# stanfordnlp/mac-network

Measured on NVIDIA H100. Metric: mac_reasoning_steps_per_sec, higher is better.
Workload: dtype bf16

## Files before the change

mac_network_b200/csrc/read_step.cuh:

```cuda
#pragma once
#include "tc_gemm.cuh"

namespace mac {

constexpr int RS_D = 512;
constexpr int RS_BM = 64;
constexpr int RS_KB = RS_D / TC_BK;
constexpr int RS_BLK = RS_BM * TC_BK * 2;
constexpr int RS_A_BYTES = RS_KB * RS_BLK;
constexpr int RS_B_HALF = 256 * TC_BK * 2;
constexpr int RS_W_BYTES = 2 * RS_B_HALF;
constexpr int RS_STAGE = RS_W_BYTES + RS_BLK;
constexpr int RS_STAGES = 2;
constexpr int RS_Q_SLOT = RS_KB;
constexpr int RS_SLOTS = RS_Q_SLOT + 1 + RS_KB;
constexpr int RS_CONSUMERS = 256;
constexpr int RS_THREADS = RS_CONSUMERS + 32;
constexpr int RS_SMEM_BYTES = RS_A_BYTES + RS_STAGES * RS_STAGE + 1024  + 64  +
                              2 * RS_BM * 4  + 2 * RS_D * 4  +
                              2 * RS_D * 4 ;
static_assert(RS_SMEM_BYTES <= 232448, "over the sm_90 per-block shared memory opt-in limit");
static_assert(RS_STAGE % 1024 == 0 && RS_W_BYTES % 1024 == 0, "swizzled operands need 1024-byte alignment");

__device__ __forceinline__ float bf16lo(uint32_t w) { return __uint_as_float(w << 16); }
__device__ __forceinline__ float bf16hi(uint32_t w) { return __uint_as_float(w & 0xffff0000u); }

__device__ __forceinline__ void wgmma_bf16_n256(float (&d)[128], uint64_t adesc, uint64_t bdesc, uint32_t accum) {
  asm volatile(
      "{\n\t.reg .pred p;\n\t"
      "setp.ne.b32 p, %130, 0;\n\t"
      "wgmma.mma_async.sync.aligned.m64n256k16.f32.bf16.bf16 "
      "{%0, %1, %2, %3, %4, %5, %6, %7, %8, %9, %10, %11, %12, %13, %14, %15, %16, %17, %18, %19, %20, %21, %22, %23, %24, %25, %26, %27, %28, %29, %30, %31, %32, %33, %34, %35, %36, %37, %38, %39, %40, %41, %42, %43, %44, %45, %46, %47, %48, %49, %50, %51, %52, %53, %54, %55, %56, %57, %58, %59, %60, %61, %62, %63, %64, %65, %66, %67, %68, %69, %70, %71, %72, %73, %74, %75, %76, %77, %78, %79, %80, %81, %82, %83, %84, %85, %86, %87, %88, %89, %90, %91, %92, %93, %94, %95, %96, %97, %98, %99, %100, %101, %102, %103, %104, %105, %106, %107, %108, %109, %110, %111, %112, %113, %114, %115, %116, %117, %118, %119, %120, %121, %122, %123, %124, %125, %126, %127}, %128, %129, p, 1, 1, 0, 0;\n\t}"
      : "+f"(d[0]), "+f"(d[1]), "+f"(d[2]), "+f"(d[3]), "+f"(d[4]), "+f"(d[5]), "+f"(d[6]), "+f"(d[7]), "+f"(d[8]), "+f"(d[9]), "+f"(d[10]), "+f"(d[11]), "+f"(d[12]), "+f"(d[13]), "+f"(d[14]), "+f"(d[15]), "+f"(d[16]), "+f"(d[17]), "+f"(d[18]), "+f"(d[19]), "+f"(d[20]), "+f"(d[21]), "+f"(d[22]), "+f"(d[23]), "+f"(d[24]), "+f"(d[25]), "+f"(d[26]), "+f"(d[27]), "+f"(d[28]), "+f"(d[29]), "+f"(d[30]), "+f"(d[31]), "+f"(d[32]), "+f"(d[33]), "+f"(d[34]), "+f"(d[35]), "+f"(d[36]), "+f"(d[37]), "+f"(d[38]), "+f"(d[39]), "+f"(d[40]), "+f"(d[41]), "+f"(d[42]), "+f"(d[43]), "+f"(d[44]), "+f"(d[45]), "+f"(d[46]), "+f"(d[47]), "+f"(d[48]), "+f"(d[49]), "+f"(d[50]), "+f"(d[51]), "+f"(d[52]), "+f"(d[53]), "+f"(d[54]), "+f"(d[55]), "+f"(d[56]), "+f"(d[57]), "+f"(d[58]), "+f"(d[59]), "+f"(d[60]), "+f"(d[61]), "+f"(d[62]), "+f"(d[63]), "+f"(d[64]), "+f"(d[65]), "+f"(d[66]), "+f"(d[67]), "+f"(d[68]), "+f"(d[69]), "+f"(d[70]), "+f"(d[71]), "+f"(d[72]), "+f"(d[73]), "+f"(d[74]), "+f"(d[75]), "+f"(d[76]), "+f"(d[77]), "+f"(d[78]), "+f"(d[79]), "+f"(d[80]), "+f"(d[81]), "+f"(d[82]), "+f"(d[83]), "+f"(d[84]), "+f"(d[85]), "+f"(d[86]), "+f"(d[87]), "+f"(d[88]), "+f"(d[89]), "+f"(d[90]), "+f"(d[91]), "+f"(d[92]), "+f"(d[93]), "+f"(d[94]), "+f"(d[95]), "+f"(d[96]), "+f"(d[97]), "+f"(d[98]), "+f"(d[99]), "+f"(d[100]), "+f"(d[101]), "+f"(d[102]), "+f"(d[103]), "+f"(d[104]), "+f"(d[105]), "+f"(d[106]), "+f"(d[107]), "+f"(d[108]), "+f"(d[109]), "+f"(d[110]), "+f"(d[111]), "+f"(d[112]), "+f"(d[113]), "+f"(d[114]), "+f"(d[115]), "+f"(d[116]), "+f"(d[117]), "+f"(d[118]), "+f"(d[119]), "+f"(d[120]), "+f"(d[121]), "+f"(d[122]), "+f"(d[123]), "+f"(d[124]), "+f"(d[125]), "+f"(d[126]), "+f"(d[127])
      : "l"(adesc), "l"(bdesc), "r"(accum));
}
inline bool read_step_supported(int B, int N, int d) {
  return d == RS_D && N >= 1 && N <= 256 && B >= 1 && B < (1 << 22);
}

struct ReadStepParams {
  int M, N;
  const float* y;
  const float* ctrl;
  const float* bm2;
  const float* wr;
  float* logits;
};

__device__ __forceinline__ void rs_consumer_bar() { asm volatile("bar.sync 1, %0;" ::"n"(RS_CONSUMERS) : "memory"); }

__global__ void __launch_bounds__(RS_THREADS, 1)
read_step_kernel(const __grid_constant__ CUtensorMap map_p, const __grid_constant__ CUtensorMap map_q,
                 const __grid_constant__ CUtensorMap map_w1, const __grid_constant__ CUtensorMap map_w2,
                 const ReadStepParams p) {
  extern __shared__ unsigned char smem_dyn[];
  const uint32_t base_u32 = smem_u32(smem_dyn);
  unsigned char* a_tile = smem_dyn + ((1024u - (base_u32 & 1023u)) & 1023u);
  unsigned char* b_ring = a_tile + RS_A_BYTES;
  uint64_t* full = reinterpret_cast<uint64_t*>(b_ring + RS_STAGES * RS_STAGE);
  uint64_t* empty = full + RS_STAGES;
  float* s_lg = reinterpret_cast<float*>(full + 8);
  float* s_ctrl = s_lg + 2 * RS_BM;
  float* s_bm2 = s_ctrl + 2 * RS_D;
  float* s_wr = s_bm2 + RS_D;

  const int warp = threadIdx.x >> 5, lane = threadIdx.x & 31;
  const int row0 = blockIdx.x * RS_BM;
  const int s_lo = row0 / p.N;

  if (threadIdx.x == RS_CONSUMERS) {
    tma_prefetch_desc(&map_p);
    tma_prefetch_desc(&map_q);
    tma_prefetch_desc(&map_w1);
    tma_prefetch_desc(&map_w2);
    for (int i = 0; i < RS_STAGES; ++i) {
      mbar_init(&full[i], 1);
      mbar_init(&empty[i], RS_CONSUMERS / 32);
    }
    fence_mbar_init();
  }
  __syncthreads();

  if (warp == RS_CONSUMERS / 32) {
    if (elect_one()) {
      for (int j = 0; j < RS_SLOTS; ++j) {
        const int s = j % RS_STAGES;
        mbar_wait(&empty[s], ((j / RS_STAGES) & 1) ^ 1);
        unsigned char* dst = b_ring + s * RS_STAGE;
        if (j == RS_Q_SLOT) {
          mbar_expect_tx(&full[s], RS_A_BYTES);
          for (int kb = 0; kb < RS_KB; ++kb) tma_load_2d(dst + kb * RS_BLK, &map_q, kb * TC_BK, row0, &full[s]);
          continue;
        }
        const bool g1 = j < RS_Q_SLOT;
        mbar_expect_tx(&full[s], g1 ? RS_W_BYTES + RS_BLK : RS_W_BYTES);
        const CUtensorMap* m = g1 ? &map_w1 : &map_w2;
        const int k0 = (g1 ? j : j - RS_Q_SLOT - 1) * TC_BK;
        if (g1) tma_load_2d(dst + RS_W_BYTES, &map_p, k0, row0, &full[s]);
        tma_load_2d(dst, m, k0, 0, &full[s]);
        tma_load_2d(dst + RS_B_HALF, m, k0, 256, &full[s]);
      }
    }
    return;
  }

  const int tid = threadIdx.x;
  const int g = warp >> 2;
  const int rl = 16 * (warp & 3) + (lane >> 2);
  const int cq = 256 * g + 2 * (lane & 3);
  const int prow = tid >> 3;
  const int poff = prow * 128 + (tid & 7) * 16;
  const int pcol = ((tid & 7) ^ (prow & 7)) << 3;
  for (int i = tid; i < RS_D; i += RS_CONSUMERS) {
    s_bm2[i] = __ldg(p.bm2 + i);
    s_wr[i] = __ldg(p.wr + i);
  }
  float acc[128];
  const int last_row = min(p.M, row0 + RS_BM) - 1;
  const int nsamp = last_row / p.N - s_lo + 1;
  for (int q = 0; q < min(nsamp, 2); ++q)
    for (int i = tid; i < RS_D; i += RS_CONSUMERS) s_ctrl[q * RS_D + i] = __ldg(p.ctrl + (size_t)(s_lo + q) * RS_D + i);
  int yoff[2];
#pragma unroll
  for (int u = 0; u < 2; ++u) yoff[u] = min(row0 + prow + 32 * u, p.M - 1) / p.N * RS_D + pcol;

  for (int j = 0; j < RS_KB; ++j) {
    const int s = j % RS_STAGES;
    unsigned char* stage = b_ring + s * RS_STAGE;
    float4 y0[2], y1[2];
#pragma unroll
    for (int u = 0; u < 2; ++u) {
      y0[u] = *reinterpret_cast<const float4*>(p.y + yoff[u] + j * TC_BK);
      y1[u] = *reinterpret_cast<const float4*>(p.y + yoff[u] + j * TC_BK + 4);
    }
    mbar_wait(&full[s], (j / RS_STAGES) & 1);
#pragma unroll
    for (int u = 0; u < 2; ++u) {
      uint4* c = reinterpret_cast<uint4*>(stage + RS_W_BYTES + poff + u * 32 * 128);
      const uint4 v = *c;
      *c = make_uint4(pack_bf16(bf16lo(v.x) * y0[u].x, bf16hi(v.x) * y0[u].y), pack_bf16(bf16lo(v.y) * y0[u].z, bf16hi(v.y) * y0[u].w),
                      pack_bf16(bf16lo(v.z) * y1[u].x, bf16hi(v.z) * y1[u].y), pack_bf16(bf16lo(v.w) * y1[u].z, bf16hi(v.w) * y1[u].w));
    }
    fence_proxy_async();
    rs_consumer_bar();
    const uint64_t adesc = make_sw128_kmajor_desc(smem_u32(stage + RS_W_BYTES));
    const uint64_t bdesc = make_sw128_kmajor_desc(smem_u32(stage + g * RS_B_HALF));
    wgmma_fence();
#pragma unroll
    for (int k = 0; k < TC_BK / 16; ++k) wgmma_bf16_n256(acc, adesc + 2 * k, bdesc + 2 * k, (j || k) ? 1u : 0u);
    wgmma_commit();
    wgmma_wait<1>();
    wgmma_hold(acc);
    if (j && lane == 0) mbar_arrive(&empty[(j - 1) % RS_STAGES]);
  }
  wgmma_wait<0>();
  wgmma_hold(acc);
  if (lane == 0) mbar_arrive(&empty[(RS_KB - 1) % RS_STAGES]);

  constexpr int qs = RS_Q_SLOT % RS_STAGES;
  const unsigned char* q_tile = b_ring + qs * RS_STAGE;
  mbar_wait(&full[qs], (RS_Q_SLOT / RS_STAGES) & 1);
#pragma unroll
  for (int h = 0; h < 2; ++h) {
    const int r = rl + 8 * h, row = row0 + r;
#pragma unroll
    for (int j = 0; j < 32; ++j) {
      const int n = cq + 8 * j;
      const int kb = n >> 6, c = (n & 63) >> 3;
      const int off = kb * RS_BLK + r * 128 + ((c ^ (r & 7)) << 4) + (n & 7) * 2;
      const uint32_t q = *reinterpret_cast<const uint32_t*>(q_tile + off);
      const uint32_t hv = row < p.M ? pack_bf16(elu_fast(acc[4 * j + 2 * h] + bf16lo(q)), elu_fast(acc[4 * j + 2 * h + 1] + bf16hi(q)))
                                    : 0u;
      *reinterpret_cast<uint32_t*>(a_tile + off) = hv;
    }
  }
  fence_proxy_async();
  rs_consumer_bar();
  if (lane == 0) mbar_arrive(&empty[qs]);

  const uint32_t a_u = smem_u32(a_tile);
  for (int j = 0; j < RS_KB; ++j) {
    const int jj = RS_Q_SLOT + 1 + j, s = jj % RS_STAGES;
    mbar_wait(&full[s], (jj / RS_STAGES) & 1);
    const uint64_t adesc = make_sw128_kmajor_desc(a_u + j * RS_BLK);
    const uint64_t bdesc = make_sw128_kmajor_desc(smem_u32(b_ring + s * RS_STAGE + g * RS_B_HALF));
    wgmma_fence();
#pragma unroll
    for (int k = 0; k < TC_BK / 16; ++k) wgmma_bf16_n256(acc, adesc + 2 * k, bdesc + 2 * k, (j || k) ? 1u : 0u);
    wgmma_commit();
    wgmma_wait<1>();
    wgmma_hold(acc);
    if (j && lane == 0) mbar_arrive(&empty[(jj - 1) % RS_STAGES]);
  }
  wgmma_wait<0>();
  wgmma_hold(acc);
  if (lane == 0) mbar_arrive(&empty[(RS_SLOTS - 1) % RS_STAGES]);

#pragma unroll
  for (int h = 0; h < 2; ++h) {
    const int r = rl + 8 * h, row = row0 + r;
    const int s = min(row, p.M - 1) / p.N;
    const float* crow = s - s_lo < 2 ? s_ctrl + (s - s_lo) * RS_D : p.ctrl + (size_t)s * RS_D;
    float part = 0.f;
#pragma unroll
    for (int j = 0; j < 32; ++j) {
      const int n = cq + 8 * j;
      const float2 cc = *reinterpret_cast<const float2*>(crow + n);
      const float2 bb = *reinterpret_cast<const float2*>(s_bm2 + n);
      const float2 ww = *reinterpret_cast<const float2*>(s_wr + n);
      const float t0 = elu_fast((acc[4 * j + 2 * h] + bb.x) * cc.x);
      const float t1 = elu_fast((acc[4 * j + 2 * h + 1] + bb.y) * cc.y);
      part = fmaf(t0, ww.x, part);
      part = fmaf(t1, ww.y, part);
    }
    part += __shfl_xor_sync(0xffffffffu, part, 1);
    part += __shfl_xor_sync(0xffffffffu, part, 2);
    if ((lane & 3) == 0) s_lg[g * RS_BM + r] = part;
  }
  rs_consumer_bar();
  if (tid < RS_BM && row0 + tid < p.M) p.logits[row0 + tid] = s_lg[tid] + s_lg[RS_BM + tid];
}

inline int read_step_launch(const void* inv, const void* kb_bf16, const float* y, const float* control,
                            const mac_read_weights* w, float* att, float* info, int B, int N, int d, cudaStream_t stream) {
  if (!read_step_supported(B, N, d)) return MAC_ERR_UNSUPPORTED;
  if (!inv || !kb_bf16 || !y || !control || !w->Wm_bf16 || !w->Wm2_bf16 || !att || !info) return MAC_ERR_INVALID;
  const int M = B * N;
  const TcReadScratch s = tc_read_scratch(const_cast<void*>(inv), B, N, d);
  CUtensorMap mp, mq, mw1, mw2;
  int st = make_tmap_2d(&mp, s.P, 1, (uint64_t)M, (uint64_t)d, (uint64_t)d * 2, RS_BM, TC_BK, 1);
  if (st != MAC_OK) return st;
  st = make_tmap_2d(&mq, s.Q, 1, (uint64_t)M, (uint64_t)d, (uint64_t)d * 2, RS_BM, TC_BK, 1);
  if (st != MAC_OK) return st;
  st = make_tmap_2d(&mw1, w->Wm_bf16, 1, (uint64_t)d, (uint64_t)d, (uint64_t)2 * d * 2, 256, TC_BK, 1);
  if (st != MAC_OK) return st;
  st = make_tmap_2d(&mw2, w->Wm2_bf16, 1, (uint64_t)d, (uint64_t)d, (uint64_t)d * 2, 256, TC_BK, 1);
  if (st != MAC_OK) return st;
  ReadStepParams p{};
  p.M = M; p.N = N; p.y = y; p.ctrl = control; p.bm2 = w->bm2; p.wr = w->wr; p.logits = s.parts;
  MAC_CUDA_TRY(cudaFuncSetAttribute(read_step_kernel, cudaFuncAttributeMaxDynamicSharedMemorySize, RS_SMEM_BYTES));
  read_step_kernel<<<(M + RS_BM - 1) / RS_BM, RS_THREADS, RS_SMEM_BYTES, stream>>>(mp, mq, mw1, mw2, p);
  MAC_LAUNCH_CHECK();
  return mac_kb_attend_fwd(s.parts, 1, w->br, kb_bf16, 1, att, info, B, N, d, stream);
}

}
```

Baseline: 17630.

## Retile fused read-step kernel to 128-row blocks with per-warpgroup rows and register rebalancing

The fused read-step GEMM kernel now handles 128 rows per block, with each consumer warpgroup owning 64 rows across all 512 output columns. Before, each warpgroup owned 256 columns of a 64-row tile, so each weight tile loaded from memory now serves twice as many rows. The P operand is loaded once into a persistent A tile with per-block barriers, and the weight ring is restaged as a 3-deep ring of 256-column halves. It adds setmaxnreg producer/consumer register reallocation, keeps the first-half hidden activations in registers, and prefetches y one step ahead. The cost is a larger block with heavy register pressure (232 registers per consumer thread), fewer blocks for small M, and control/bias/weight vectors read from global memory instead of shared memory.

```diff
diff --git a/mac_network_b200/csrc/read_step.cuh b/mac_network_b200/csrc/read_step.cuh
--- a/mac_network_b200/csrc/read_step.cuh
+++ b/mac_network_b200/csrc/read_step.cuh
@@ -9,18 +9,31 @@
 constexpr int RS_BLK = RS_BM * TC_BK * 2;
 constexpr int RS_A_BYTES = RS_KB * RS_BLK;
 constexpr int RS_B_HALF = 256 * TC_BK * 2;
-constexpr int RS_W_BYTES = 2 * RS_B_HALF;
-constexpr int RS_STAGE = RS_W_BYTES + RS_BLK;
-constexpr int RS_STAGES = 2;
-constexpr int RS_Q_SLOT = RS_KB;
-constexpr int RS_SLOTS = RS_Q_SLOT + 1 + RS_KB;
 constexpr int RS_CONSUMERS = 256;
 constexpr int RS_THREADS = RS_CONSUMERS + 32;
-constexpr int RS_SMEM_BYTES = RS_A_BYTES + RS_STAGES * RS_STAGE + 1024  + 64  +
-                              2 * RS_BM * 4  + 2 * RS_D * 4  +
-                              2 * RS_D * 4 ;
-static_assert(RS_SMEM_BYTES <= 232448, "over the sm_90 per-block shared memory opt-in limit");
-static_assert(RS_STAGE % 1024 == 0 && RS_W_BYTES % 1024 == 0, "swizzled operands need 1024-byte alignment");
+
+constexpr int RS128_BM = 128;
+constexpr int RS128_BLK = RS128_BM * TC_BK * 2;
+constexpr int RS128_A_BYTES = RS_KB * RS128_BLK;
+constexpr int RS128_STAGE = RS_B_HALF;
+constexpr int RS128_STAGES = 3;
+constexpr int RS128_Q0 = RS_KB;
+constexpr int RS128_G1B = RS128_Q0 + 2;
+constexpr int RS128_Q1 = RS128_G1B + RS_KB;
+constexpr int RS128_G2A = RS128_Q1 + 2;
+constexpr int RS128_G2B = RS128_G2A + RS_KB;
+constexpr int RS128_SLOTS = RS128_G2B + RS_KB;
+constexpr int RS128_CONSUMERS = 256;
+constexpr int RS128_THREADS = RS128_CONSUMERS + 128;
+constexpr int RS128_SMEM_BYTES = RS128_A_BYTES + RS128_STAGES * RS128_STAGE + 1024  +
+                                 8 * (RS_KB + 2 * RS128_STAGES) ;
+static_assert(RS128_SMEM_BYTES <= 232448, "over the sm_90 per-block shared memory opt-in limit");
+static_assert(RS128_BLK % 1024 == 0 && RS128_STAGE % 1024 == 0 && (RS128_BM / 2) * 128 % 1024 == 0,
+              "swizzled operands need 1024-byte alignment");
+static_assert(2 * RS128_BLK == RS128_STAGE, "a ring slot holds two Q blocks");
+constexpr int RS128_PRODUCER_REGS = 40;
+constexpr int RS128_CONSUMER_REGS = 232;
+static_assert(RS128_PRODUCER_REGS + 2 * RS128_CONSUMER_REGS <= 3 * (65536 / RS128_THREADS / 8 * 8), "register budget");
 
 __device__ __forceinline__ float bf16lo(uint32_t w) { return __uint_as_float(w << 16); }
 __device__ __forceinline__ float bf16hi(uint32_t w) { return __uint_as_float(w & 0xffff0000u); }
@@ -49,176 +62,232 @@
 
 __device__ __forceinline__ void rs_consumer_bar() { asm volatile("bar.sync 1, %0;" ::"n"(RS_CONSUMERS) : "memory"); }
 
-__global__ void __launch_bounds__(RS_THREADS, 1)
+__device__ __forceinline__ void rs128_wg_bar(int g) { asm volatile("bar.sync %0, 128;" ::"r"(1 + g) : "memory"); }
+
+__device__ __forceinline__ void rs128_gemm_half(float (&acc)[128], uint32_t a_u, uint32_t ring_u, uint64_t* full,
+                                                uint64_t* empty, int t0, int lane) {
+  for (int j = 0; j < RS_KB; ++j) {
+    const int t = t0 + j, s = t % RS128_STAGES;
+    mbar_wait(&full[s], (t / RS128_STAGES) & 1);
+    const uint64_t adesc = make_sw128_kmajor_desc(a_u + j * RS128_BLK);
+    const uint64_t bdesc = make_sw128_kmajor_desc(ring_u + s * RS128_STAGE);
+    wgmma_fence();
+#pragma unroll
+    for (int k = 0; k < TC_BK / 16; ++k) wgmma_bf16_n256(acc, adesc + 2 * k, bdesc + 2 * k, (j || k) ? 1u : 0u);
+    wgmma_commit();
+    wgmma_wait<1>();
+    wgmma_hold(acc);
+    if (j && lane == 0) mbar_arrive(&empty[(t - 1) % RS128_STAGES]);
+  }
+  wgmma_wait<0>();
+  wgmma_hold(acc);
+  if (lane == 0) mbar_arrive(&empty[(t0 + RS_KB - 1) % RS128_STAGES]);
+}
+
+__device__ __forceinline__ int rs128_sw_off(int r, int n, int blk) {
+  return (n >> 6) * blk + r * 128 + ((((n & 63) >> 3) ^ (r & 7)) << 4) + (n & 7) * 2;
+}
+
+__global__ void __launch_bounds__(RS128_THREADS, 1)
 read_step_kernel(const __grid_constant__ CUtensorMap map_p, const __grid_constant__ CUtensorMap map_q,
                  const __grid_constant__ CUtensorMap map_w1, const __grid_constant__ CUtensorMap map_w2,
                  const ReadStepParams p) {
   extern __shared__ unsigned char smem_dyn[];
   const uint32_t base_u32 = smem_u32(smem_dyn);
   unsigned char* a_tile = smem_dyn + ((1024u - (base_u32 & 1023u)) & 1023u);
-  unsigned char* b_ring = a_tile + RS_A_BYTES;
-  uint64_t* full = reinterpret_cast<uint64_t*>(b_ring + RS_STAGES * RS_STAGE);
-  uint64_t* empty = full + RS_STAGES;
-  float* s_lg = reinterpret_cast<float*>(full + 8);
-  float* s_ctrl = s_lg + 2 * RS_BM;
-  float* s_bm2 = s_ctrl + 2 * RS_D;
-  float* s_wr = s_bm2 + RS_D;
+  unsigned char* ring = a_tile + RS128_A_BYTES;
+  uint64_t* pfull = reinterpret_cast<uint64_t*>(ring + RS128_STAGES * RS128_STAGE);
+  uint64_t* full = pfull + RS_KB;
+  uint64_t* empty = full + RS128_STAGES;
 
   const int warp = threadIdx.x >> 5, lane = threadIdx.x & 31;
-  const int row0 = blockIdx.x * RS_BM;
-  const int s_lo = row0 / p.N;
-
-  if (threadIdx.x == RS_CONSUMERS) {
+  const int row0 = blockIdx.x * RS128_BM;
+
+  if (threadIdx.x == RS128_CONSUMERS) {
     tma_prefetch_desc(&map_p);
     tma_prefetch_desc(&map_q);
     tma_prefetch_desc(&map_w1);
     tma_prefetch_desc(&map_w2);
-    for (int i = 0; i < RS_STAGES; ++i) {
+    for (int i = 0; i < RS_KB; ++i) mbar_init(&pfull[i], 1);
+    for (int i = 0; i < RS128_STAGES; ++i) {
       mbar_init(&full[i], 1);
-      mbar_init(&empty[i], RS_CONSUMERS / 32);
+      mbar_init(&empty[i], RS128_CONSUMERS / 32);
     }
     fence_mbar_init();
   }
   __syncthreads();
 
-  if (warp == RS_CONSUMERS / 32) {
-    if (elect_one()) {
-      for (int j = 0; j < RS_SLOTS; ++j) {
-        const int s = j % RS_STAGES;
-        mbar_wait(&empty[s], ((j / RS_STAGES) & 1) ^ 1);
-        unsigned char* dst = b_ring + s * RS_STAGE;
-        if (j == RS_Q_SLOT) {
-          mbar_expect_tx(&full[s], RS_A_BYTES);
-          for (int kb = 0; kb < RS_KB; ++kb) tma_load_2d(dst + kb * RS_BLK, &map_q, kb * TC_BK, row0, &full[s]);
-          continue;
+  if (warp >= RS128_CONSUMERS / 32) {
+    asm volatile("setmaxnreg.dec.sync.aligned.u32 %0;" ::"n"(RS128_PRODUCER_REGS));
+    if (warp == RS128_CONSUMERS / 32 && elect_one()) {
+      auto load_p = [&](int j) {
+        mbar_expect_tx(&pfull[j], RS128_BLK);
+        tma_load_2d(a_tile + j * RS128_BLK, &map_p, j * TC_BK, row0, &pfull[j]);
+      };
+      for (int t = 0; t < RS128_SLOTS; ++t) {
+        if (t < RS128_STAGES) load_p(t);
+        else if (t == RS128_STAGES)
+          for (int j = RS128_STAGES; j < RS_KB; ++j) load_p(j);
+        const int s = t % RS128_STAGES;
+        mbar_wait(&empty[s], ((t / RS128_STAGES) & 1) ^ 1);
+        unsigned char* dst = ring + s * RS128_STAGE;
+        mbar_expect_tx(&full[s], RS128_STAGE);
+        if (t < RS128_G2A) {
+          const int half = t >= RS128_G1B, u = t - half * RS128_G1B;
+          if (u < RS_KB) {
+            tma_load_2d(dst, &map_w1, u * TC_BK, 256 * half, &full[s]);
+          } else {
+            const int kb = 4 * half + 2 * (u - RS_KB);
+            tma_load_2d(dst, &map_q, kb * TC_BK, row0, &full[s]);
+            tma_load_2d(dst + RS128_BLK, &map_q, (kb + 1) * TC_BK, row0, &full[s]);
+          }
+        } else {
+          const int half = t >= RS128_G2B, u = t - (half ? RS128_G2B : RS128_G2A);
+          tma_load_2d(dst, &map_w2, u * TC_BK, 256 * half, &full[s]);
         }
-        const bool g1 = j < RS_Q_SLOT;
-        mbar_expect_tx(&full[s], g1 ? RS_W_BYTES + RS_BLK : RS_W_BYTES);
-        const CUtensorMap* m = g1 ? &map_w1 : &map_w2;
-        const int k0 = (g1 ? j : j - RS_Q_SLOT - 1) * TC_BK;
-        if (g1) tma_load_2d(dst + RS_W_BYTES, &map_p, k0, row0, &full[s]);
-        tma_load_2d(dst, m, k0, 0, &full[s]);
-        tma_load_2d(dst + RS_B_HALF, m, k0, 256, &full[s]);
       }
     }
     return;
   }
 
-  const int tid = threadIdx.x;
+  asm volatile("setmaxnreg.inc.sync.aligned.u32 %0;" ::"n"(RS128_CONSUMER_REGS));
   const int g = warp >> 2;
+  const int wt = threadIdx.x & 127;
   const int rl = 16 * (warp & 3) + (lane >> 2);
-  const int cq = 256 * g + 2 * (lane & 3);
-  const int prow = tid >> 3;
-  const int poff = prow * 128 + (tid & 7) * 16;
-  const int pcol = ((tid & 7) ^ (prow & 7)) << 3;
-  for (int i = tid; i < RS_D; i += RS_CONSUMERS) {
-    s_bm2[i] = __ldg(p.bm2 + i);
-    s_wr[i] = __ldg(p.wr + i);
-  }
+  const int cq = 2 * (lane & 3);
+  const int rowg = row0 + 64 * g;
+  unsigned char* a_wg = a_tile + g * (RS128_BM / 2) * 128;
+  const uint32_t a_u = smem_u32(a_wg), ring_u = smem_u32(ring);
+  const int prow = wt >> 3;
+  const int poff = prow * 128 + (wt & 7) * 16;
+  const int pcol = ((wt & 7) ^ (prow & 7)) << 3;
+  int yoff[4];
+#pragma unroll
+  for (int u = 0; u < 4; ++u) yoff[u] = min(rowg + prow + 16 * u, p.M - 1) / p.N * RS_D + pcol;
+
   float acc[128];
-  const int last_row = min(p.M, row0 + RS_BM) - 1;
-  const int nsamp = last_row / p.N - s_lo + 1;
-  for (int q = 0; q < min(nsamp, 2); ++q)
-    for (int i = tid; i < RS_D; i += RS_CONSUMERS) s_ctrl[q * RS_D + i] = __ldg(p.ctrl + (size_t)(s_lo + q) * RS_D + i);
-  int yoff[2];
-#pragma unroll
-  for (int u = 0; u < 2; ++u) yoff[u] = min(row0 + prow + 32 * u, p.M - 1) / p.N * RS_D + pcol;
-
-  for (int j = 0; j < RS_KB; ++j) {
-    const int s = j % RS_STAGES;
-    unsigned char* stage = b_ring + s * RS_STAGE;
-    float4 y0[2], y1[2];
-#pragma unroll
-    for (int u = 0; u < 2; ++u) {
+  float4 y0[4], y1[4];
+  auto load_y = [&](int j) {
+#pragma unroll
+    for (int u = 0; u < 4; ++u) {
       y0[u] = *reinterpret_cast<const float4*>(p.y + yoff[u] + j * TC_BK);
       y1[u] = *reinterpret_cast<const float4*>(p.y + yoff[u] + j * TC_BK + 4);
     }
-    mbar_wait(&full[s], (j / RS_STAGES) & 1);
-#pragma unroll
-    for (int u = 0; u < 2; ++u) {
-      uint4* c = reinterpret_cast<uint4*>(stage + RS_W_BYTES + poff + u * 32 * 128);
+  };
+  load_y(0);
+  for (int j = 0; j < RS_KB; ++j) {
+    const int s = j % RS128_STAGES;
+    mbar_wait(&pfull[j], 0);
+#pragma unroll
+    for (int u = 0; u < 4; ++u) {
+      uint4* c = reinterpret_cast<uint4*>(a_wg + j * RS128_BLK + poff + u * 16 * 128);
       const uint4 v = *c;
       *c = make_uint4(pack_bf16(bf16lo(v.x) * y0[u].x, bf16hi(v.x) * y0[u].y), pack_bf16(bf16lo(v.y) * y0[u].z, bf16hi(v.y) * y0[u].w),
                       pack_bf16(bf16lo(v.z) * y1[u].x, bf16hi(v.z) * y1[u].y), pack_bf16(bf16lo(v.w) * y1[u].z, bf16hi(v.w) * y1[u].w));
     }
     fence_proxy_async();
-    rs_consumer_bar();
-    const uint64_t adesc = make_sw128_kmajor_desc(smem_u32(stage + RS_W_BYTES));
-    const uint64_t bdesc = make_sw128_kmajor_desc(smem_u32(stage + g * RS_B_HALF));
+    rs128_wg_bar(g);
+    mbar_wait(&full[s], (j / RS128_STAGES) & 1);
+    const uint64_t adesc = make_sw128_kmajor_desc(a_u + j * RS128_BLK);
+    const uint64_t bdesc = make_sw128_kmajor_desc(ring_u + s * RS128_STAGE);
     wgmma_fence();
 #pragma unroll
     for (int k = 0; k < TC_BK / 16; ++k) wgmma_bf16_n256(acc, adesc + 2 * k, bdesc + 2 * k, (j || k) ? 1u : 0u);
     wgmma_commit();
+    if (j + 1 < RS_KB) load_y(j + 1);
     wgmma_wait<1>();
     wgmma_hold(acc);
-    if (j && lane == 0) mbar_arrive(&empty[(j - 1) % RS_STAGES]);
+    if (j && lane == 0) mbar_arrive(&empty[(j - 1) % RS128_STAGES]);
   }
   wgmma_wait<0>();
   wgmma_hold(acc);
-  if (lane == 0) mbar_arrive(&empty[(RS_KB - 1) % RS_STAGES]);
-
-  constexpr int qs = RS_Q_SLOT % RS_STAGES;
-  const unsigned char* q_tile = b_ring + qs * RS_STAGE;
-  mbar_wait(&full[qs], (RS_Q_SLOT / RS_STAGES) & 1);
+  if (lane == 0) mbar_arrive(&empty[(RS_KB - 1) % RS128_STAGES]);
+
+  uint32_t h0[64];
+#pragma unroll
+  for (int q = 0; q < 2; ++q) {
+    const int t = RS128_Q0 + q, s = t % RS128_STAGES;
+    mbar_wait(&full[s], (t / RS128_STAGES) & 1);
+    const unsigned char* q_tile = ring + s * RS128_STAGE + g * (RS128_BM / 2) * 128 - 2 * q * RS128_BLK;
+#pragma unroll
+    for (int h = 0; h < 2; ++h) {
+      const int r = rl + 8 * h;
+      const bool live = rowg + r < p.M;
+#pragma unroll
+      for (int j = 16 * q; j < 16 * q + 16; ++j) {
+        const uint32_t qv = *reinterpret_cast<const uint32_t*>(q_tile + rs128_sw_off(r, cq + 8 * j, RS128_BLK));
+        h0[2 * j + h] = live ? pack_bf16(elu_fast(acc[4 * j + 2 * h] + bf16lo(qv)), elu_fast(acc[4 * j + 2 * h + 1] + bf16hi(qv)))
+                             : 0u;
+      }
+    }
+    __syncwarp();
+    if (lane == 0) mbar_arrive(&empty[s]);
+  }
+
+  rs128_gemm_half(acc, a_u, ring_u, full, empty, RS128_G1B, lane);
+
+  rs128_wg_bar(g);
 #pragma unroll
   for (int h = 0; h < 2; ++h) {
-    const int r = rl + 8 * h, row = row0 + r;
-#pragma unroll
-    for (int j = 0; j < 32; ++j) {
-      const int n = cq + 8 * j;
-      const int kb = n >> 6, c = (n & 63) >> 3;
-      const int off = kb * RS_BLK + r * 128 + ((c ^ (r & 7)) << 4) + (n & 7) * 2;
-      const uint32_t q = *reinterpret_cast<const uint32_t*>(q_tile + off);
-      const uint32_t hv = row < p.M ? pack_bf16(elu_fast(acc[4 * j + 2 * h] + bf16lo(q)), elu_fast(acc[4 * j + 2 * h + 1] + bf16hi(q)))
-                                    : 0u;
-      *reinterpret_cast<uint32_t*>(a_tile + off) = hv;
-    }
+    const int r = rl + 8 * h;
+#pragma unroll
+    for (int j = 0; j < 32; ++j) *reinterpret_cast<uint32_t*>(a_wg + rs128_sw_off(r, cq + 8 * j, RS128_BLK)) = h0[2 * j + h];
+  }
+#pragma unroll
+  for (int q = 0; q < 2; ++q) {
+    const int t = RS128_Q1 + q, s = t % RS128_STAGES;
+    mbar_wait(&full[s], (t / RS128_STAGES) & 1);
+    const unsigned char* q_tile = ring + s * RS128_STAGE + g * (RS128_BM / 2) * 128 - 2 * q * RS128_BLK;
+#pragma unroll
+    for (int h = 0; h < 2; ++h) {
+      const int r = rl + 8 * h;
+      const bool live = rowg + r < p.M;
+#pragma unroll
+      for (int j = 16 * q; j < 16 * q + 16; ++j) {
+        const int n = cq + 8 * j;
+        const uint32_t qv = *reinterpret_cast<const uint32_t*>(q_tile + rs128_sw_off(r, n, RS128_BLK));
+        *reinterpret_cast<uint32_t*>(a_wg + rs128_sw_off(r, 256 + n, RS128_BLK)) =
+            live ? pack_bf16(elu_fast(acc[4 * j + 2 * h] + bf16lo(qv)), elu_fast(acc[4 * j + 2 * h + 1] + bf16hi(qv))) : 0u;
+      }
+    }
+    __syncwarp();
+    if (lane == 0) mbar_arrive(&empty[s]);
   }
   fence_proxy_async();
-  rs_consumer_bar();
-  if (lane == 0) mbar_arrive(&empty[qs]);
-
-  const uint32_t a_u = smem_u32(a_tile);
-  for (int j = 0; j < RS_KB; ++j) {
-    const int jj = RS_Q_SLOT + 1 + j, s = jj % RS_STAGES;
-    mbar_wait(&full[s], (jj / RS_STAGES) & 1);
-    const uint64_t adesc = make_sw128_kmajor_desc(a_u + j * RS_BLK);
-    const uint64_t bdesc = make_sw128_kmajor_desc(smem_u32(b_ring + s * RS_STAGE + g * RS_B_HALF));
-    wgmma_fence();
-#pragma unroll
-    for (int k = 0; k < TC_BK / 16; ++k) wgmma_bf16_n256(acc, adesc + 2 * k, bdesc + 2 * k, (j || k) ? 1u : 0u);
-    wgmma_commit();
-    wgmma_wait<1>();
-    wgmma_hold(acc);
-    if (j && lane == 0) mbar_arrive(&empty[(jj - 1) % RS_STAGES]);
-  }
-  wgmma_wait<0>();
-  wgmma_hold(acc);
-  if (lane == 0) mbar_arrive(&empty[(RS_SLOTS - 1) % RS_STAGES]);
-
+  rs128_wg_bar(g);
+
+  float part[2][2];
+#pragma unroll
+  for (int half = 0; half < 2; ++half) {
+    rs128_gemm_half(acc, a_u, ring_u, full, empty, half ? RS128_G2B : RS128_G2A, lane);
+#pragma unroll
+    for (int h = 0; h < 2; ++h) {
+      const int row = rowg + rl + 8 * h;
+      const float* crow = p.ctrl + (size_t)(min(row, p.M - 1) / p.N) * RS_D + 256 * half;
+      const float* bm2 = p.bm2 + 256 * half;
+      const float* wr = p.wr + 256 * half;
+      float s = 0.f;
+#pragma unroll
+      for (int j = 0; j < 32; ++j) {
+        const int n = cq + 8 * j;
+        const float2 cc = __ldg(reinterpret_cast<const float2*>(crow + n));
+        const float2 bb = __ldg(reinterpret_cast<const float2*>(bm2 + n));
+        const float2 ww = __ldg(reinterpret_cast<const float2*>(wr + n));
+        const float t0 = elu_fast((acc[4 * j + 2 * h] + bb.x) * cc.x);
+        const float t1 = elu_fast((acc[4 * j + 2 * h + 1] + bb.y) * cc.y);
+        s = fmaf(t0, ww.x, s);
+        s = fmaf(t1, ww.y, s);
+      }
+      s += __shfl_xor_sync(0xffffffffu, s, 1);
+      s += __shfl_xor_sync(0xffffffffu, s, 2);
+      part[half][h] = s;
+    }
+  }
 #pragma unroll
   for (int h = 0; h < 2; ++h) {
-    const int r = rl + 8 * h, row = row0 + r;
-    const int s = min(row, p.M - 1) / p.N;
-    const float* crow = s - s_lo < 2 ? s_ctrl + (s - s_lo) * RS_D : p.ctrl + (size_t)s * RS_D;
-    float part = 0.f;
-#pragma unroll
-    for (int j = 0; j < 32; ++j) {
-      const int n = cq + 8 * j;
-      const float2 cc = *reinterpret_cast<const float2*>(crow + n);
-      const float2 bb = *reinterpret_cast<const float2*>(s_bm2 + n);
-      const float2 ww = *reinterpret_cast<const float2*>(s_wr + n);
-      const float t0 = elu_fast((acc[4 * j + 2 * h] + bb.x) * cc.x);
-      const float t1 = elu_fast((acc[4 * j + 2 * h + 1] + bb.y) * cc.y);
-      part = fmaf(t0, ww.x, part);
-      part = fmaf(t1, ww.y, part);
-    }
-    part += __shfl_xor_sync(0xffffffffu, part, 1);
-    part += __shfl_xor_sync(0xffffffffu, part, 2);
-    if ((lane & 3) == 0) s_lg[g * RS_BM + r] = part;
-  }
-  rs_consumer_bar();
-  if (tid < RS_BM && row0 + tid < p.M) p.logits[row0 + tid] = s_lg[tid] + s_lg[RS_BM + tid];
+    const int row = rowg + rl + 8 * h;
+    if ((lane & 3) == 0 && row < p.M) p.logits[row] = part[0][h] + part[1][h];
+  }
 }
 
 inline int read_step_launch(const void* inv, const void* kb_bf16, const float* y, const float* control,
@@ -228,9 +297,9 @@
   const int M = B * N;
   const TcReadScratch s = tc_read_scratch(const_cast<void*>(inv), B, N, d);
   CUtensorMap mp, mq, mw1, mw2;
-  int st = make_tmap_2d(&mp, s.P, 1, (uint64_t)M, (uint64_t)d, (uint64_t)d * 2, RS_BM, TC_BK, 1);
+  int st = make_tmap_2d(&mp, s.P, 1, (uint64_t)M, (uint64_t)d, (uint64_t)d * 2, RS128_BM, TC_BK, 1);
   if (st != MAC_OK) return st;
-  st = make_tmap_2d(&mq, s.Q, 1, (uint64_t)M, (uint64_t)d, (uint64_t)d * 2, RS_BM, TC_BK, 1);
+  st = make_tmap_2d(&mq, s.Q, 1, (uint64_t)M, (uint64_t)d, (uint64_t)d * 2, RS128_BM, TC_BK, 1);
   if (st != MAC_OK) return st;
   st = make_tmap_2d(&mw1, w->Wm_bf16, 1, (uint64_t)d, (uint64_t)d, (uint64_t)2 * d * 2, 256, TC_BK, 1);
   if (st != MAC_OK) return st;
@@ -238,8 +307,8 @@
   if (st != MAC_OK) return st;
   ReadStepParams p{};
   p.M = M; p.N = N; p.y = y; p.ctrl = control; p.bm2 = w->bm2; p.wr = w->wr; p.logits = s.parts;
-  MAC_CUDA_TRY(cudaFuncSetAttribute(read_step_kernel, cudaFuncAttributeMaxDynamicSharedMemorySize, RS_SMEM_BYTES));
-  read_step_kernel<<<(M + RS_BM - 1) / RS_BM, RS_THREADS, RS_SMEM_BYTES, stream>>>(mp, mq, mw1, mw2, p);
+  MAC_CUDA_TRY(cudaFuncSetAttribute(read_step_kernel, cudaFuncAttributeMaxDynamicSharedMemorySize, RS128_SMEM_BYTES));
+  read_step_kernel<<<(M + RS128_BM - 1) / RS128_BM, RS128_THREADS, RS128_SMEM_BYTES, stream>>>(mp, mq, mw1, mw2, p);
   MAC_LAUNCH_CHECK();
   return mac_kb_attend_fwd(s.parts, 1, w->br, kb_bf16, 1, att, info, B, N, d, stream);
 }
diff --git a/profiles/read_step_128.py b/profiles/read_step_128.py
--- /dev/null
+++ b/profiles/read_step_128.py
@@ -0,0 +1,103 @@
+import argparse
+import json
+import os
+import shutil
+import subprocess
+import sys
+import tempfile
+
+import numpy as np
+
+ROOT = os.path.dirname(os.path.dirname(os.path.abspath(__file__)))
+LIB_REL = os.path.join("mac_network_b200", "csrc", "libmac_b200.so")
+SIDES = ("base", "new")
+
+
+def device_info():
+    q = subprocess.run(["nvidia-smi", "--query-gpu=name,power.limit,clocks.max.sm", "--format=csv,noheader"],
+                       capture_output=True, text=True, timeout=60)
+    name, power, clock = [s.strip() for s in q.stdout.strip().splitlines()[0].split(",")]
+    return {"name": name, "power_limit": power, "max_sm_clock": clock}
+
+
+def spread(xs):
+    xs = [float(x) for x in xs]
+    return {"median": float(np.median(xs)), "min": min(xs), "max": max(xs), "runs": [round(x, 3) for x in xs]}
+
+
+def tree_copy(dst, lib):
+    shutil.copytree(ROOT, dst, ignore=shutil.ignore_patterns(".git", "*.o", "__pycache__"))
+    shutil.copyfile(lib, os.path.join(dst, LIB_REL))
+    return dst
+
+
+def bench(tree, extra, timeout_s=1800):
+    out = subprocess.run([sys.executable, os.path.join(tree, "bench.py")] + extra, capture_output=True, text=True,
+                         timeout=timeout_s, cwd=tree)
+    if out.returncode != 0:
+        raise RuntimeError("bench.py %s: exit %d: %s" % (" ".join(extra), out.returncode, out.stderr[-2000:]))
+    line = json.loads(out.stdout.strip().splitlines()[-1])
+    print("%s %s: %s" % (os.path.basename(tree), " ".join(extra), line.get("value", "done")), flush=True)
+    return line
+
+
+def main():
+    ap = argparse.ArgumentParser()
+    ap.add_argument("out_dir")
+    ap.add_argument("--base-lib", required=True)
+    ap.add_argument("--runs", type=int, default=3)
+    ap.add_argument("--roof-runs", type=int, default=6)
+    ap.add_argument("--part", default="both", choices=["rooflines", "headline", "both"])
+    args = ap.parse_args()
+    out = {"device": device_info(), "runs": args.runs, "roof_runs": args.roof_runs,
+           "headline_args": "--gpus 1 --steps 480 --warmup 12 --skip-cpu"}
+    tmp = tempfile.mkdtemp(prefix="read_step_128_")
+    try:
+        trees = {"base": tree_copy(os.path.join(tmp, "base"), os.path.abspath(args.base_lib)),
+                 "new": tree_copy(os.path.join(tmp, "new"), os.path.join(ROOT, LIB_REL))}
+        dumps = {s: os.path.join(tmp, "dump_" + s) for s in SIDES}
+
+        roof = {s: [] for s in SIDES}
+        for _ in range(args.roof_runs if args.part != "headline" else 0):
+            for s in SIDES:
+                roof[s].append(bench(trees[s], ["--rooflines-only"])["read_step_fused"]["us"])
+        if args.part != "headline":
+            out["read_step_fused_us"] = {s: spread(roof[s]) for s in SIDES}
+            out["read_step_fused_speedup"] = (out["read_step_fused_us"]["base"]["median"] /
+                                              out["read_step_fused_us"]["new"]["median"])
+        if args.part == "rooflines":
+            return finish(args, out)
+
+        lines = {s: {"headline": [], "bf16_gqa": [], "batched_one_stream": [], "batched_two_streams": []} for s in SIDES}
+        for i in range(args.runs):
+            for s in SIDES:
+                extra = ["--gpus", "1", "--steps", "480", "--warmup", "12", "--skip-cpu"]
+                line = bench(trees[s], extra + (["--dump-outputs", dumps[s]] if i == 0 else []))
+                lines[s]["headline"].append(line["value"])
+                lines[s]["bf16_gqa"].append(line["sub_lines"]["bf16_gqa"]["value"])
+                lines[s]["batched_one_stream"].append(line["info_batched_requests"]["requests_x6_one_stream"]["value"])
+                lines[s]["batched_two_streams"].append(line["info_batched_requests"]["requests_x6_two_streams"]["value"])
+        out["reasoning_steps_per_s"] = {s: {k: spread(v) for k, v in lines[s].items()} for s in SIDES}
+        out["headline_speedup"] = (out["reasoning_steps_per_s"]["new"]["headline"]["median"] /
+                                   out["reasoning_steps_per_s"]["base"]["headline"]["median"])
+
+        same = {}
+        for name in sorted(os.listdir(dumps["base"])):
+            a, b = np.load(os.path.join(dumps["base"], name)), np.load(os.path.join(dumps["new"], name))
+            same[name] = bool(a.shape == b.shape and a.dtype == b.dtype and a.tobytes() == b.tobytes())
+        out["outputs_bit_identical"] = same
+    finally:
+        shutil.rmtree(tmp, ignore_errors=True)
+    finish(args, out)
+
+
+def finish(args, out):
+    os.makedirs(args.out_dir, exist_ok=True)
+    path = os.path.join(args.out_dir, "read_step_128_%s_h100.json" % args.part)
+    with open(path, "w") as f:
+        json.dump(out, f, indent=1)
+    print(json.dumps(out))
+
+
+if __name__ == "__main__":
+    main()
```

After: 19390, median of 6. +10.0%, better.
